# MatteoBattilana/CUDAVideoStream

Hardware: AMD Instinct MI355X
Metric: 1920×1080 RGB24 frames/sec (diff+threshold+pack); achieved HBM GB/s vs peak (higher is better)
Workload: dtype u8

## Files before the change

### cudavideostream_amd/csrc/core.hip

```cpp
#include <cmath>
#include <cstdio>
#include <cstdlib>
#include <cstring>
#include <new>
#include <string>
#include <vector>

#include "../../include/mi355diff.h"
#include "cwire_common.h"

using namespace mi355;

static inline size_t code_chunks(size_t max_batch) { return (max_batch + 2) / 3 + 1; }

namespace {

thread_local std::string g_err;

int fail(int code, const char *what, hipError_t e = hipSuccess) {
    char buf[512];
    if (e != hipSuccess)
        snprintf(buf, sizeof buf, "%s: %s (%s)", what, hipGetErrorName(e), hipGetErrorString(e));
    else
        snprintf(buf, sizeof buf, "%s", what);
    g_err = buf;
    return code;
}

#define HIP_TRY(expr)                                             \
    do {                                                          \
        hipError_t _e = (expr);                                   \
        if (_e != hipSuccess) return fail(MI355_ERR_HIP, #expr, _e); \
    } while (0)

}

struct mi355_core {
    mi355_config cfg{};
    int device = 0;
    uint32_t n = 0;
    uint32_t ntiles = 0;
    hipStream_t own_stream = nullptr;
    hipStream_t stream = nullptr;

    uint8_t *state = nullptr, *in = nullptr, *aux = nullptr, *vis = nullptr;
    uint4 *rec = nullptr, *meta = nullptr;
    uint32_t *codes = nullptr;
    uint32_t *groff = nullptr, *totals = nullptr;
    uint64_t scan_epoch = 0;
    uint32_t *offsets = nullptr;
    int32_t *one_xs = nullptr;
    uint8_t *one_diff = nullptr;
    int32_t *hist = nullptr, *thr = nullptr;
    uint32_t *red_bounds = nullptr;
    uint32_t *cw_cnt = nullptr;
    uint8_t *cw_rec = nullptr;
    uint64_t *cw_rec_pos = nullptr;
    uint64_t cw_rec_bytes = 0;
    static constexpr int kRecWords = 4;
    uint32_t *h_rec = nullptr;
    bool cw_warm = false;
    uint4 *cw_items = nullptr;
    uint32_t *cw_esc = nullptr;
    CwaFrame *cwa_ftab = nullptr;
    uint4 *cwa_chunk = nullptr;
    uint4 *cwa_dir = nullptr;
    uint32_t *cwb_hist = nullptr;
    uint8_t *gray1 = nullptr;
    size_t gray1_stride = 0;
    float *k9 = nullptr;
    float *kxk = nullptr;
    uint8_t *lut = nullptr;
    uint8_t *glyphs = nullptr;
    int nglyphs = 0, glyph_h = 0, glyph_w = 0;
    std::string charset;
    bool have_k9 = false, k9_sym = false;
    size_t workspace = 0;

    uint32_t *h_count = nullptr;

    static constexpr int kMaxSlots = 8;
    struct Slot {
        uint8_t *d_in = nullptr, *d_vis = nullptr;
        uint32_t *h_count = nullptr;
        hipEvent_t uploaded = nullptr, painted = nullptr, packed = nullptr, shown = nullptr;
        bool has_vis = false;
        bool compact = false;
        int64_t ticket = -1;
    };
    Slot slots[kMaxSlots];
    int nslots = 0;
    int64_t next_ticket = 0;
    hipStream_t up_stream = nullptr, down_stream = nullptr;

    struct LogSet {
        uint4 *rec = nullptr, *meta = nullptr;
        uint32_t *codes = nullptr, *groff = nullptr, *totals = nullptr;
        hipEvent_t packed = nullptr, expanded = nullptr;
        bool in_use = false;
    };
    static constexpr int kSets = 2;
    LogSet set[kSets];
    int flip = 0;
    hipStream_t side = nullptr;
    hipEvent_t side_done = nullptr;
    bool pipeline_ok = true;
    int median_rows = 0;
    uint32_t cu_count = 0;
    hipStream_t main2 = nullptr;
    hipEvent_t packed2[kSets] = {};
    static constexpr uint32_t kDensePct = 40;
    uint64_t *h_tot = nullptr;
    bool dense = false;
    bool filter_since_batch = false;
    hipEvent_t fork[kSets] = {};
    int parts_pending = -1;
    const void *fb_states = nullptr;
    size_t fb_stride = 0;

    static constexpr int kEvRing = 32, kEvPer = 6;
    bool timing = false;
    hipEvent_t ev[kEvRing][kEvPer] = {};
    bool ev_split[kEvRing] = {};
    int ev_head = 0, ev_count = 0;
    double ms_pack = 0, ms_scan = 0, ms_expand = 0, ms_total = 0;
    int launches = 0;
};

namespace mi355 {
int set_error(int code, const char *what) { return fail(code, what); }
hipStream_t core_stream(::mi355_core *c) {
    if (c->side_done && hipSetDevice(c->device) == hipSuccess && hipStreamWaitEvent(c->stream, c->side_done, 0) == hipSuccess)
        c->side_done = nullptr;
    return c->stream;
}
int core_device(const ::mi355_core *c) { return c->device; }
}

namespace {

hipError_t make_stream(const mi355_core *c, hipStream_t *s) {
    if (c->cfg.flags & MI355_FLAG_OWN_QUEUES) {
        int least = 0, greatest = 0;
        if (hipDeviceGetStreamPriorityRange(&least, &greatest) == hipSuccess && least != greatest)
            return hipStreamCreateWithPriority(s, hipStreamNonBlocking, least);
        (void)hipGetLastError();
    }
    return hipStreamCreateWithFlags(s, hipStreamNonBlocking);
}

template <class T>
int dev_alloc(mi355_core *c, T **p, size_t count) {
    const size_t bytes = count * sizeof(T);
    HIP_TRY(hipMalloc((void **)p, bytes ? bytes : 16));
    c->workspace += bytes;
    return MI355_OK;
}

int use_device(mi355_core *c, bool join = true, bool parts = true) {
    HIP_TRY(hipSetDevice(c->device));
    if (join && c->side_done) {
        HIP_TRY(hipStreamWaitEvent(c->stream, c->side_done, 0));
        c->side_done = nullptr;
        c->parts_pending = -1;
    }
    if (parts && c->parts_pending >= 0) {
        HIP_TRY(hipStreamWaitEvent(c->stream, c->packed2[c->parts_pending], 0));
        c->parts_pending = -1;
    }
    return MI355_OK;
}

int use_device_filter(mi355_core *c) {
    c->filter_since_batch = true;
    return use_device(c, false);
}

int harvest_timing(mi355_core *c, int keep = 0) {
    while (c->ev_count > keep) {
        hipEvent_t *e = c->ev[c->ev_head];
        HIP_TRY(hipEventSynchronize(e[4]));
        float a = 0, b = 0, d = 0, t = 0;
        HIP_TRY(hipEventElapsedTime(&a, e[0], e[1]));
        if (c->ev_split[c->ev_head]) {
            float a2 = 0;
            HIP_TRY(hipEventElapsedTime(&a2, e[0], e[5]));
            a = a2 > a ? a2 : a;
        }
        HIP_TRY(hipEventElapsedTime(&b, e[2], e[3]));
        HIP_TRY(hipEventElapsedTime(&d, e[3], e[4]));
        HIP_TRY(hipEventElapsedTime(&t, e[0], e[4]));
        c->ms_pack += a;
        c->ms_scan += b;
        c->ms_expand += d;
        c->ms_total += t;
        c->launches += 1;
        c->ev_head = (c->ev_head + 1) % mi355_core::kEvRing;
        c->ev_count -= 1;
    }
    return MI355_OK;
}

void build_heat_lut(uint8_t *lut) {
    for (int diff = 0; diff <= 765; diff++) {
        float diff1 = diff / (255.0 * 2.0);
        double r = sin(M_PI * diff1 - M_PI / 2.0) * 255.0;
        double g = sin(M_PI * diff1) * 255.0;
        double b = sin(M_PI * diff1 + M_PI / 2.0) * 255.0;
        r = r > 0.0 ? r : 0.0; r = r < 255.0 ? r : 255.0;
        g = g > 0.0 ? g : 0.0; g = g < 255.0 ? g : 255.0;
        b = b > 0.0 ? b : 0.0; b = b < 255.0 ? b : 255.0;
        lut[diff * 3 + 0] = (uint8_t)(int)b;
        lut[diff * 3 + 1] = (uint8_t)(int)g;
        lut[diff * 3 + 2] = (uint8_t)(int)r;
    }
}

int need_gray1(mi355_core *c) {
    if (c->gray1 || c->n == 0) return MI355_OK;
    c->gray1_stride = ((size_t)c->n / 3 + 15) & ~(size_t)15;
    return dev_alloc(c, &c->gray1, c->gray1_stride * (size_t)c->cfg.max_batch);
}

int clear_totals(mi355_core *c) {
    const size_t bytes = 2 * (size_t)c->cfg.max_batch * sizeof(uint32_t);
    HIP_TRY(hipMemsetAsync(c->totals, 0, bytes, c->stream));
    if (c->set[1].totals) HIP_TRY(hipMemsetAsync(c->set[1].totals, 0, bytes, c->stream));
    HIP_TRY(hipStreamSynchronize(c->stream));
    return MI355_OK;
}

int need_red_bounds(mi355_core *c) {
    if (c->red_bounds || c->n == 0) return MI355_OK;
    return dev_alloc(c, &c->red_bounds, (size_t)c->cfg.max_batch * red_bounds_per_frame(c->n));
}

int setup_pipeline(mi355_core *c) {
    if (c->side || !c->pipeline_ok) return MI355_OK;
    const size_t T = (size_t)c->cfg.max_batch, W = c->ntiles;
    mi355_core::LogSet &s0 = c->set[0], &s1 = c->set[1];
    s0.rec = c->rec; s0.codes = c->codes; s0.meta = c->meta; s0.groff = c->groff; s0.totals = c->totals;
    bool ok = true;
    ok = ok && hipMalloc((void **)&s1.rec, T * W * 1024) == hipSuccess;
    ok = ok && hipMalloc((void **)&s1.codes, code_chunks(T) * W * 1024) == hipSuccess;
    ok = ok && hipMalloc((void **)&s1.meta, T * W * 16) == hipSuccess;
    ok = ok && hipMalloc((void **)&s1.groff, T * expand_groups(c->ntiles) * 16) == hipSuccess;
    ok = ok && hipMalloc((void **)&s1.totals, (2 * T + 2) * sizeof(uint32_t)) == hipSuccess;
    ok = ok && hipMemsetAsync(s1.totals, 0, (2 * T + 2) * sizeof(uint32_t), c->stream) == hipSuccess &&
         hipStreamSynchronize(c->stream) == hipSuccess;
    ok = ok && make_stream(c, &c->side) == hipSuccess;
    ok = ok && make_stream(c, &c->main2) == hipSuccess;
    for (int i = 0; i < mi355_core::kSets && ok; i++) {
        const unsigned flags = hipEventDisableTiming | hipEventReleaseToDevice;
        ok = hipEventCreateWithFlags(&c->set[i].packed, flags) == hipSuccess &&
             hipEventCreateWithFlags(&c->set[i].expanded, flags) == hipSuccess &&
             hipEventCreateWithFlags(&c->packed2[i], flags) == hipSuccess &&
             hipEventCreateWithFlags(&c->fork[i], flags) == hipSuccess;
    }
    if (!ok) {
        (void)hipGetLastError();
        void *ptrs[] = {s1.rec, s1.codes, s1.meta, s1.groff, s1.totals};
        for (void *p : ptrs) if (p) (void)hipFree(p);
        s1.rec = nullptr; s1.meta = nullptr; s1.codes = s1.groff = s1.totals = nullptr;
        if (c->side) { (void)hipStreamDestroy(c->side); c->side = nullptr; }
        if (c->main2) { (void)hipStreamDestroy(c->main2); c->main2 = nullptr; }
        for (int i = 0; i < mi355_core::kSets; i++) {
            hipEvent_t *evs[] = {&c->set[i].packed, &c->set[i].expanded, &c->packed2[i], &c->fork[i]};
            for (hipEvent_t *e : evs) if (*e) { (void)hipEventDestroy(*e); *e = nullptr; }
        }
        c->pipeline_ok = false;
        return MI355_OK;
    }
    c->workspace += T * W * 1024 + code_chunks(T) * W * 1024 + T * W * 16 + T * expand_groups(c->ntiles) * 16 + (2 * T + 2) * 4;
    return MI355_OK;
}

struct CwireOut {
    uint64_t *frame_pos;
    uint8_t *cwire;
    uint64_t capacity;
};

CwireDirectArgs cwire_args(mi355_core *c, const CwireOut *cw, const uint32_t *d_offsets, uint32_t ntiles) {
    CwireDirectArgs x{};
    x.x.offsets = d_offsets;
    x.x.ntiles = ntiles;
    x.items = c->cw_items;
    x.esc = c->cw_esc;
    x.frame_pos = cw->frame_pos;
    x.cwire = cw->cwire;
    x.capacity = cw->capacity;
    return x;
}

int run_batch(mi355_core *c, bool pair, const void *d_cur, const void *d_prev, size_t stride,
              int nframes, void *d_offsets, void *d_xs, void *d_diff, size_t capacity,
              void *d_wire = nullptr, bool pipelined = false, const CwireOut *cw = nullptr, bool feedback = false,
              int seg = 0) {
    if (!c) return fail(MI355_ERR_INVALID, "null core");
    if (nframes < 0 || nframes > c->cfg.max_batch)
        return fail(MI355_ERR_INVALID, "nframes outside [0, max_batch]");
    if (!d_offsets) return fail(MI355_ERR_INVALID, "null d_offsets");
    if (nframes > 0 && c->n > 0 && (!d_cur || (pair && !d_prev)))
        return fail(MI355_ERR_INVALID, "null frame pointer");
    if (nframes > 0 && stride < c->n) return fail(MI355_ERR_INVALID, "stride_bytes < frame bytes");
    if (capacity > 0 && !d_wire && !cw && (!d_xs || !d_diff)) return fail(MI355_ERR_INVALID, "null output pointer");
    pipelined = pipelined && c->stream == c->own_stream && c->pipeline_ok && nframes > 0 && c->n > 0;
    const bool own = pipelined;
    if (c->filter_since_batch) pipelined = false;
    c->filter_since_batch = false;
    if (pipelined) {
        const bool same_states = feedback && c->fb_states == d_prev && c->fb_stride == stride;
        if (int rc = use_device(c, false, !same_states && (feedback || c->fb_states))) return rc;
        if (int rc = setup_pipeline(c)) return rc;
        pipelined = c->pipeline_ok;
    }
    if (pipelined && c->h_tot) {
        const uint64_t note = __atomic_load_n(c->h_tot, __ATOMIC_RELAXED);
        if (note >> 32) c->dense = (note & 0xffffffffull) * 100u > (uint64_t)mi355_core::kDensePct * (note >> 32) * c->n;
        if (c->dense) pipelined = false;
    }
    if (!pipelined)
        if (int rc = use_device(c)) return rc;
    c->fb_states = nullptr;
    if (nframes == 0 || c->n == 0) {
        HIP_TRY(hipMemsetAsync(d_offsets, 0, sizeof(uint32_t) * ((size_t)nframes + 1), c->stream));
        if (d_wire) {
            const size_t head = 4 * (size_t)nframes < capacity ? 4 * (size_t)nframes : capacity & ~(size_t)3;
            if (head) HIP_TRY(hipMemsetAsync(d_wire, 0, head, c->stream));
        }
        if (cw) HIP_TRY(launch_expand_cwire(cwire_args(c, cw, (const uint32_t *)d_offsets, 0u), nframes, c->stream));
        return MI355_OK;
    }
    hipEvent_t *tev = nullptr;
    if (c->timing) {
        if (int rc = harvest_timing(c, mi355_core::kEvRing - 1)) return rc;
        tev = c->ev[(c->ev_head + c->ev_count) % mi355_core::kEvRing];
    }
    mi355_core::LogSet one;
    one.rec = c->rec; one.codes = c->codes; one.meta = c->meta; one.groff = c->groff; one.totals = c->totals;
    mi355_core::LogSet &ls = pipelined ? c->set[c->flip] : one;
    hipStream_t tail = pipelined ? c->side : c->stream;
    if (pipelined && ls.in_use) HIP_TRY(hipStreamWaitEvent(c->stream, ls.expanded, 0));
    if (tev) HIP_TRY(hipEventRecord(tev[0], c->stream));
    PackArgs a{};
    a.cur = (const uint8_t *)d_cur;
    a.prev = seg ? nullptr : (const uint8_t *)d_prev;
    a.state = c->state;
    a.seg = seg;
    if (seg) a.states = (uint8_t *)const_cast<void *>(d_prev);
    a.stride = stride;
    a.n = c->n;
    a.nframes = nframes;
    a.thr = c->cfg.threshold;
    a.ntiles = c->ntiles;
    a.tile_begin = 0;
    a.tile_end = c->ntiles;
    a.rec = ls.rec;
    a.codes = ls.codes;
    a.codes_bytes = (uint32_t)(code_chunks((size_t)c->cfg.max_batch) * c->ntiles * 1024u);
    a.meta = ls.meta;
    a.rec_bytes = (uint32_t)((size_t)c->cfg.max_batch * c->ntiles * 1024u);
    a.meta_bytes = (uint32_t)((size_t)c->cfg.max_batch * c->ntiles * 16u);
    const bool aligned = (((uintptr_t)d_cur | (uintptr_t)d_prev | stride) & 15u) == 0 && 3 * (uint64_t)stride + c->n < (1ull << 32);
    bool pair_once = false;
    if (pair) {
        const int64_t d = (int64_t)((intptr_t)d_prev - (intptr_t)d_cur), st = (int64_t)stride, T = nframes;
        bool shared = false;
        const int64_t k0 = d / st;
        for (int64_t k = k0 - 1; k <= k0 + 1; k++)
            if (k > -T && k < T && (d - k * st < 0 ? k * st - d : d - k * st) < (int64_t)c->n) shared = true;
        pair_once = !shared;
    }
    const uint32_t k1_blocks = 4u * c->cu_count;
    const bool split = pipelined && c->main2 && c->ntiles >= 64;
    if (split) {
        const uint32_t cut = (c->ntiles / 2) & ~3u;
        uint32_t blocks0 = 0, blocks1 = 0;
        if (k1_blocks) {
            blocks0 = (uint32_t)((uint64_t)k1_blocks * cut / c->ntiles);
            if (blocks0 == 0) blocks0 = 1;
            blocks1 = k1_blocks > blocks0 ? k1_blocks - blocks0 : 1u;
        }
        HIP_TRY(hipEventRecord(c->fork[c->flip], c->stream));
        PackArgs a0 = a, a1 = a;
        a0.tile_end = cut;
        a1.tile_begin = cut;
        HIP_TRY(launch_diff_pack(a0, pair, aligned, pair_once, blocks0, c->stream, feedback));
        HIP_TRY(hipStreamWaitEvent(c->main2, c->fork[c->flip], 0));
        if (ls.in_use) HIP_TRY(hipStreamWaitEvent(c->main2, ls.expanded, 0));
        HIP_TRY(launch_diff_pack(a1, pair, aligned, pair_once, blocks1, c->main2, feedback));
        HIP_TRY(hipEventRecord(c->packed2[c->flip], c->main2));
        HIP_TRY(hipStreamWaitEvent(tail, c->packed2[c->flip], 0));
        if (tev) HIP_TRY(hipEventRecord(tev[5], c->main2));
        c->parts_pending = c->flip;
        if (feedback) { c->fb_states = d_prev; c->fb_stride = stride; }
    } else {
        HIP_TRY(launch_diff_pack(a, pair, aligned, pair_once, pipelined ? k1_blocks : 0u, c->stream, feedback));
    }
    if (tev) {
        HIP_TRY(hipEventRecord(tev[1], c->stream));
        c->ev_split[(c->ev_head + c->ev_count) % mi355_core::kEvRing] = split;
    }
    if (pipelined) {
        HIP_TRY(hipEventRecord(ls.packed, c->stream));
        HIP_TRY(hipStreamWaitEvent(tail, ls.packed, 0));
    }
    if (tev) HIP_TRY(hipEventRecord(tev[2], tail));
    if (next_scan_epoch(c->scan_epoch)) {
        HIP_TRY(hipStreamSynchronize(c->stream));
        if (c->side) HIP_TRY(hipStreamSynchronize(c->side));
        if (c->main2) HIP_TRY(hipStreamSynchronize(c->main2));
        if (int rc = clear_totals(c)) return rc;
    }
    uint64_t *const note = own && c->h_tot && c->pipeline_ok ? c->h_tot : nullptr;
    HIP_TRY(launch_scan(ls.meta, ls.groff, (uint64_t *)ls.totals, c->ntiles, nframes, (uint32_t *)d_offsets,
                        ls.totals + 2 * (size_t)c->cfg.max_batch, c->scan_epoch, note, tail));
    if (tev) HIP_TRY(hipEventRecord(tev[3], tail));
    ExpandArgs g{};
    g.rec = ls.rec;
    g.codes = ls.codes;
    g.meta = ls.meta;
    g.roff = ls.groff;
    g.offsets = (const uint32_t *)d_offsets;
    g.ntiles = c->ntiles;
    g.codes_bytes = a.codes_bytes;
    g.rec_bytes = a.rec_bytes;
    g.out_xs = (int32_t *)d_xs;
    g.out_diff = (uint8_t *)d_diff;
    g.wire = (uint8_t *)d_wire;
    g.capacity = capacity;
    if (cw) {
        CwireDirectArgs x = cwire_args(c, cw, g.offsets, c->ntiles);
        x.x = g;
        HIP_TRY(launch_expand_cwire(x, nframes, tail));
    } else {
        HIP_TRY(launch_expand(g, nframes, tail));
    }
    if (tev) {
        HIP_TRY(hipEventRecord(tev[4], tail));
        c->ev_count += 1;
    }
    if (pipelined) {
        HIP_TRY(hipEventRecord(ls.expanded, tail));
        ls.in_use = true;
        c->side_done = ls.expanded;
        c->flip ^= 1;
    }
    return MI355_OK;
}

}

extern "C" {

const char *mi355_last_error(void) { return g_err.c_str(); }

int mi355_abi_version(void) { return MI355_ABI_VERSION; }

int mi355_create(const mi355_config *cfg, mi355_core **out) {
    if (!cfg || !out) return fail(MI355_ERR_INVALID, "null argument");
    *out = nullptr;
    if (cfg->width < 0 || cfg->height < 0) return fail(MI355_ERR_INVALID, "negative frame size");
    if (cfg->threshold < 0 || cfg->threshold > 255) return fail(MI355_ERR_INVALID, "threshold outside 0..255");
    if (cfg->max_batch < 1) return fail(MI355_ERR_INVALID, "max_batch < 1");
    if (cfg->visualizer < 0 || cfg->visualizer > 5) return fail(MI355_ERR_INVALID, "unknown visualizer");
    if (cfg->flags & ~MI355_FLAG_OWN_QUEUES) return fail(MI355_ERR_INVALID, "flags: unknown bit (MI355_FLAG_OWN_QUEUES is the only flag of this version of the library)");
    const uint64_t n64 = 3ull * (uint64_t)cfg->width * (uint64_t)cfg->height;
    if (n64 >= (1ull << 31)) return fail(MI355_ERR_INVALID, "frame larger than 2 GiB");
    {
        const uint64_t tiles = (n64 + kTileBytes - 1) / kTileBytes, mb = (uint64_t)cfg->max_batch;
        const uint64_t chunks = mb > code_chunks((size_t)mb) ? mb : (uint64_t)code_chunks((size_t)mb);
        if (tiles * kTileBytes * chunks >= (1ull << 32))
            return fail(MI355_ERR_INVALID, "max_batch * frame bytes must stay below 2^32");
    }

    int ndev = 0;
    hipError_t e = hipGetDeviceCount(&ndev);
    if (e != hipSuccess || ndev <= 0)
        return fail(MI355_ERR_HIP, "no HIP device available (libmi355diff has no CPU fallback)", e);
    mi355_core *c = new (std::nothrow) mi355_core;
    if (!c) return fail(MI355_ERR_INVALID, "out of host memory");
    c->cfg = *cfg;
    if (const char *v = getenv("MI355_PIPELINE")) c->pipeline_ok = v[0] != '0';
    if (cfg->device >= 0) c->device = cfg->device;
    else if ((e = hipGetDevice(&c->device)) != hipSuccess) { delete c; return fail(MI355_ERR_HIP, "hipGetDevice", e); }
    if (c->device >= ndev) { delete c; return fail(MI355_ERR_INVALID, "device ordinal out of range"); }

    c->n = (uint32_t)n64;
    c->ntiles = (c->n + kTileBytes - 1) / kTileBytes;
    {
        hipDeviceProp_t prop{};
        if (hipGetDeviceProperties(&prop, c->device) == hipSuccess && prop.multiProcessorCount > 0) c->cu_count = (uint32_t)prop.multiProcessorCount;
    }
    const size_t T = (size_t)cfg->max_batch, W = c->ntiles, N = c->n;

    int rc = use_device(c);
    if (!rc) { e = make_stream(c, &c->own_stream); if (e != hipSuccess) rc = fail(MI355_ERR_HIP, "hipStreamCreate", e); }
    c->stream = c->own_stream;
    for (int i = 0; i < mi355_core::kEvRing * mi355_core::kEvPer && !rc; i++) { e = hipEventCreateWithFlags(&c->ev[i / mi355_core::kEvPer][i % mi355_core::kEvPer], hipEventDisableSystemFence); if (e != hipSuccess) rc = fail(MI355_ERR_HIP, "hipEventCreate", e); }
    if (!rc && (e = init_gray_table()) != hipSuccess) rc = fail(MI355_ERR_HIP, "init_gray_table", e);
    if (!rc) rc = dev_alloc(c, &c->state, N + 16);
    if (!rc) rc = dev_alloc(c, &c->in, N + 16);
    if (!rc) rc = dev_alloc(c, &c->aux, N + 16);
    if (!rc) rc = dev_alloc(c, &c->vis, N + 16);
    if (!rc) rc = dev_alloc(c, &c->rec, T * W * 64);
    if (!rc) rc = dev_alloc(c, &c->codes, code_chunks(T) * W * 256);
    if (!rc) rc = dev_alloc(c, &c->meta, T * W);
    if (!rc) rc = dev_alloc(c, &c->groff, T * expand_groups(c->ntiles) * 4);
    if (!rc) rc = dev_alloc(c, &c->totals, 2 * T + 2);
    if (!rc) { e = hipMemsetAsync(c->totals, 0, (2 * T + 2) * sizeof(uint32_t), c->own_stream); if (e != hipSuccess) rc = fail(MI355_ERR_HIP, "hipMemset", e); }
    if (!rc) rc = dev_alloc(c, &c->offsets, T + 1);
    if (!rc) rc = dev_alloc(c, &c->cw_cnt, (size_t)kCwireSlots);
    if (!rc) rc = dev_alloc(c, &c->cw_items, T * cwire_items_per_frame(c->ntiles));
    if (!rc) rc = dev_alloc(c, &c->cw_esc, T);
    if (!rc) rc = dev_alloc(c, &c->cwa_ftab, T);
    if (!rc) rc = dev_alloc(c, &c->cwa_chunk, T * cwa_chunks(c->n));
    if (!rc) rc = dev_alloc(c, &c->cwa_dir, T * cwa_tiles(c->n));
    if (!rc) rc = dev_alloc(c, &c->cwb_hist, T * kCwbWords);
    if (!rc) rc = dev_alloc(c, &c->one_xs, N + 4);
    if (!rc) rc = dev_alloc(c, &c->one_diff, N + 16);
    if (!rc) rc = dev_alloc(c, &c->hist, 256 * T);
    if (!rc) rc = dev_alloc(c, &c->thr, T);
    if (!rc) rc = dev_alloc(c, &c->k9, 9);
    if (!rc) rc = dev_alloc(c, &c->lut, 768 * 3);
    if (!rc) { e = hipHostMalloc((void **)&c->h_count, 2 * sizeof(uint32_t), hipHostMallocDefault); if (e != hipSuccess) rc = fail(MI355_ERR_HIP, "hipHostMalloc", e); }
    if (!rc) { e = hipHostMalloc((void **)&c->h_tot, sizeof(uint64_t), hipHostMallocDefault); if (e != hipSuccess) rc = fail(MI355_ERR_HIP, "hipHostMalloc", e); else *c->h_tot = 0; }
    if (!rc) { e = hipMemsetAsync(c->state, 0, N + 16, c->own_stream); if (e != hipSuccess) rc = fail(MI355_ERR_HIP, "hipMemset", e); }
    if (!rc) { e = hipStreamSynchronize(c->own_stream); if (e != hipSuccess) rc = fail(MI355_ERR_HIP, "hipStreamSynchronize", e); }
    if (!rc) {
        uint8_t lut[768 * 3] = {0};
        build_heat_lut(lut);
        e = hipMemcpy(c->lut, lut, sizeof lut, hipMemcpyHostToDevice);
        if (e != hipSuccess) rc = fail(MI355_ERR_HIP, "hipMemcpy(lut)", e);
    }
    if (!rc && cfg->visualizer == MI355_VIS_BINARIZE) rc = need_gray1(c);
    if (rc) { mi355_destroy(c); return rc; }
    *out = c;
    return MI355_OK;
}

void mi355_destroy(mi355_core *c) {
    if (!c) return;
    (void)hipSetDevice(c->device);
    if (c->nslots) (void)mi355_pipe_close(c);
    if (c->side) (void)hipStreamSynchronize(c->side);
    if (c->own_stream) (void)hipStreamSynchronize(c->own_stream);
    {
        mi355_core::LogSet &s1 = c->set[1];
        void *more[] = {s1.rec, s1.codes, s1.meta, s1.groff, s1.totals};
        for (void *p : more) if (p) (void)hipFree(p);
        for (auto &ls : c->set) {
            if (ls.packed) (void)hipEventDestroy(ls.packed);
            if (ls.expanded) (void)hipEventDestroy(ls.expanded);
        }
        if (c->side) (void)hipStreamDestroy(c->side);
        if (c->main2) { (void)hipStreamSynchronize(c->main2); (void)hipStreamDestroy(c->main2); }
        for (auto &e : c->packed2) if (e) (void)hipEventDestroy(e);
        for (auto &e : c->fork) if (e) (void)hipEventDestroy(e);
        if (c->h_tot) (void)hipHostFree(c->h_tot);
    }
    void *ptrs[] = {c->state, c->in, c->aux, c->vis, c->rec, c->codes, c->meta, c->groff, c->totals, c->offsets, c->one_xs, c->one_diff, c->hist, c->thr, c->k9,
                    c->lut, c->glyphs, c->kxk, c->gray1, c->red_bounds, c->cw_cnt, c->cw_items, c->cw_esc,
                    c->cwa_ftab, c->cwa_chunk, c->cwa_dir, c->cwb_hist, c->cw_rec, c->cw_rec_pos};
    for (void *p : ptrs) if (p) (void)hipFree(p);
    if (c->h_count) (void)hipHostFree(c->h_count);
    if (c->h_rec) (void)hipHostFree(c->h_rec);
    for (auto &slot : c->ev) for (auto &ev : slot) if (ev) (void)hipEventDestroy(ev);
    if (c->own_stream) (void)hipStreamDestroy(c->own_stream);
    delete c;
}

static int warm_exec(mi355_core *c);
static int need_exec_cwire(mi355_core *c);

int mi355_prepare(mi355_core *c, unsigned what) {
    if (!c) return fail(MI355_ERR_INVALID, "null core");
    if (what & ~(MI355_PREPARE_ALL | MI355_PREPARE_EXEC_CWIRE)) return fail(MI355_ERR_INVALID, "mi355_prepare: unknown bit in `what`");
    if (int rc = use_device(c)) return rc;
    if ((what & MI355_PREPARE_BATCHES) && c->n > 0) {
        if (int rc = setup_pipeline(c)) return rc;
    }
    if (what & MI355_PREPARE_GRAY_CHAIN)
        if (int rc = need_gray1(c)) return rc;
    if (what & MI355_PREPARE_RED_CLEAR)
        if (int rc = need_red_bounds(c)) return rc;
    if ((what & MI355_PREPARE_CONV_KXK) && !c->kxk)
        if (int rc = dev_alloc(c, &c->kxk, 81)) return rc;
    if ((what & MI355_PREPARE_EXEC) && c->n > 0 && c->nslots == 0)
        if (int rc = warm_exec(c)) return rc;
    if (what & MI355_PREPARE_EXEC_CWIRE)
        if (int rc = need_exec_cwire(c)) return rc;
    HIP_TRY(hipDeviceSynchronize());
    return MI355_OK;
}

size_t mi355_frame_bytes(const mi355_core *c) { return c ? c->n : 0; }
size_t mi355_workspace_bytes(const mi355_core *c) { return c ? c->workspace : 0; }

int mi355_set_stream(mi355_core *c, void *hip_stream) {
    if (!c) return fail(MI355_ERR_INVALID, "null core");
    if (int rc = use_device(c)) return rc;
    if (int rc = harvest_timing(c)) return rc;
    HIP_TRY(hipStreamSynchronize(c->stream));
    c->stream = (hipStream_t)hip_stream;
    return MI355_OK;
}

int mi355_use_own_stream(mi355_core *c) {
    if (!c) return fail(MI355_ERR_INVALID, "null core");
    if (int rc = use_device(c)) return rc;
    if (int rc = harvest_timing(c)) return rc;
    HIP_TRY(hipStreamSynchronize(c->stream));
    c->stream = c->own_stream;
    return MI355_OK;
}

int mi355_synchronize(mi355_core *c) {
    if (!c) return fail(MI355_ERR_INVALID, "null core");
    if (int rc = use_device(c)) return rc;
    HIP_TRY(hipStreamSynchronize(c->stream));
    return MI355_OK;
}

int mi355_set_option(mi355_core *c, int option, int value) {
    if (!c) return fail(MI355_ERR_INVALID, "null core");
    if (int rc = use_device(c)) return rc;
    HIP_TRY(hipStreamSynchronize(c->stream));
    switch (option) {
        case MI355_OPT_PIPELINE:
            if (value != 0 && value != 1) return fail(MI355_ERR_INVALID, "MI355_OPT_PIPELINE: 0 or 1");
            c->pipeline_ok = value == 1;
            return MI355_OK;
        case MI355_OPT_MEDIAN_ROWS:
            if (value < 0 || value > 60 || value % 5) return fail(MI355_ERR_INVALID, "MI355_OPT_MEDIAN_ROWS: 0 (default) or 5, 10, .. 60");
            c->median_rows = value;
            return MI355_OK;
        case MI355_OPT_SCAN_EPOCH_LEFT:
            if (value < 1 || value > (1 << 30)) return fail(MI355_ERR_INVALID, "MI355_OPT_SCAN_EPOCH_LEFT: 1..2^30");
            if (c->side) HIP_TRY(hipStreamSynchronize(c->side));
            if (c->main2) HIP_TRY(hipStreamSynchronize(c->main2));
            if (int rc = clear_totals(c)) return rc;
            c->scan_epoch = kEpochWrap - 1 - (uint64_t)value;
            return MI355_OK;
        default: return fail(MI355_ERR_INVALID, "unknown option");
    }
}

int mi355_get_option(mi355_core *c, int option, int *value) {
    if (!c || !value) return fail(MI355_ERR_INVALID, "null argument");
    switch (option) {
        case MI355_OPT_PIPELINE: *value = c->pipeline_ok ? 1 : 0; return MI355_OK;
        case MI355_OPT_MEDIAN_ROWS: *value = c->median_rows; return MI355_OK;
        case MI355_OPT_SCAN_EPOCH_LEFT: {
            const uint64_t left = kEpochWrap - 1 - c->scan_epoch;
            *value = left > (1ull << 30) ? (1 << 30) : (int)left;
            return MI355_OK;
        }
        default: return fail(MI355_ERR_INVALID, "unknown option");
    }
// ... 1818 lines not shown
```

### cudavideostream_amd/csrc/diff_pack.hip

```cpp
#include <cstdio>
#include <vector>

#include "cwire_common.h"
#include "pack_common.h"

namespace mi355 {

constexpr int kStreamPrefetch = 4;
template <bool PAIR>
struct PrefetchOf { static constexpr int value = PAIR ? 2 : kStreamPrefetch; };
static_assert(kStreamPrefetch % 2 == 0, "frames are processed in pairs");

typedef uint32_t u32x4 __attribute__((ext_vector_type(4)));
constexpr uint32_t kRsrcWord3 = 0x00020000u;
constexpr uint32_t kOOB = 0xFFFFFFFFu;

__device__ __forceinline__ __amdgpu_buffer_rsrc_t make_rsrc(const void *p, uint32_t bytes) {
    return __builtin_amdgcn_make_buffer_rsrc(const_cast<void *>(p), 0, (int)bytes, (int)kRsrcWord3);
}

struct LogOut {
    __amdgpu_buffer_rsrc_t codes, recs, meta;
};

constexpr int kStateLoadAux = 0, kStateStoreAux = 2;

template <bool HIGH>
__device__ __forceinline__ void compare_step(const uint4 c, uint4 &s, ThrConst tc, uint32_t (&dm)[4], uint32_t &m16) {
    const uint32_t cw[4] = {c.x, c.y, c.z, c.w};
    uint32_t sw[4] = {s.x, s.y, s.z, s.w};
    uint32_t fh[4];
#pragma unroll
    for (int k = 0; k < 4; k++) {
        uint32_t x;
        fh[k] = dword_flags<HIGH>(cw[k], sw[k], tc, x);
        const uint32_t mask = __builtin_amdgcn_perm(0u, 0u, fh[k]);
        dm[k] = bytes_sub_from_x(cw[k], sw[k], x, tc.h) & mask;
        sw[k] = bitop3<(TA & TC) | (TB & ~TC)>(cw[k], sw[k], mask);
    }
    s = make_uint4(sw[0], sw[1], sw[2], sw[3]);
    const uint32_t lo = __builtin_amdgcn_udot4(fh[1], tc.w1, __builtin_amdgcn_udot4(fh[0], tc.w0, 0u, false), false);
    const uint32_t hi = __builtin_amdgcn_udot4(fh[3], tc.w1, __builtin_amdgcn_udot4(fh[2], tc.w0, 0u, false), false);
    m16 = (lo + (hi << 8)) >> 7;
}

struct LogPos {
    uint32_t ptrC, roomC, ptrM, roomM;
};

__device__ __forceinline__ uint32_t emit_step(const uint32_t (&dm)[4], uint32_t m16, const LogOut &lg, LogPos &lp,
                                              uint32_t jump, uint32_t lane24, uint32_t &pc, uint32_t &pm) {
    const bool cand = m16 != 0u;
    const bool multi = (m16 & (m16 - 1u)) != 0u;
    const uint64_t bc = __ballot(cand), bm = __ballot(multi);
    const uint32_t rankC = __builtin_amdgcn_mbcnt_hi((uint32_t)(bc >> 32), __builtin_amdgcn_mbcnt_lo((uint32_t)bc, 0u));
    const uint32_t rankM = __builtin_amdgcn_mbcnt_hi((uint32_t)(bm >> 32), __builtin_amdgcn_mbcnt_lo((uint32_t)bm, 0u));
    const uint32_t nc = (uint32_t)__builtin_popcountll(bc), nm = (uint32_t)__builtin_popcountll(bm);
    pc = lp.ptrC;
    pm = lp.ptrM;
    if (nc == 0u) return 0u;
    if (nm > lp.roomM) { lp.ptrM += lp.roomM * 16u + jump; lp.roomM = 64u; }
    pm = lp.ptrM;
    if (nm == 64u) {
        const u32x4 v = {dm[0], dm[1], dm[2], dm[3]};
        __builtin_amdgcn_raw_buffer_store_b128(v, lg.recs, pm + rankM * 16u, 0, 0);
        lp.ptrM += 64u * 16u;
        lp.roomM -= 64u;
        return 64u | (64u << 16);
    }
    if (nc > lp.roomC) { lp.ptrC += lp.roomC * 4u + jump; lp.roomC = 256u; }
    pc = lp.ptrC;
    const uint32_t one = __builtin_amdgcn_sad_u8((dm[0] | dm[1]) | (dm[2] | dm[3]), 0u, 0u);
    const uint32_t code = m16 | ((multi ? rankM : one) << 16) | lane24;
    __builtin_amdgcn_raw_buffer_store_b32(code, lg.codes, cand ? pc + rankC * 4u : kOOB, 0, 0);
    const u32x4 v = {dm[0], dm[1], dm[2], dm[3]};
    __builtin_amdgcn_raw_buffer_store_b128(v, lg.recs, multi ? pm + rankM * 16u : kOOB, 0, 0);
    lp.ptrC += nc * 4u;
    lp.roomC -= nc;
    lp.ptrM += nm * 16u;
    lp.roomM -= nm;
    return nc | (nm << 16);
}

template <bool PAIR, bool FAST>
struct Group {
    static constexpr int kPrefetch = PrefetchOf<PAIR>::value;
    uint4 c[kPrefetch];
    uint4 p[kPrefetch];

    template <bool ONCE, bool FB = false>
    __device__ __forceinline__ void load_desc(__amdgpu_buffer_rsrc_t cur, __amdgpu_buffer_rsrc_t prev, const uint32_t (&voff)[kPrefetch]) {
#pragma unroll
        for (int d = 0; d < kPrefetch; d++) {
            const u32x4 v = __builtin_amdgcn_raw_buffer_load_b128(cur, voff[d], 0, ONCE ? 2 : 0);
            c[d] = make_uint4(v.x, v.y, v.z, v.w);
            if (PAIR) {
                const u32x4 w = __builtin_amdgcn_raw_buffer_load_b128(prev, voff[d], 0, FB ? kStateLoadAux : (ONCE ? 2 : 0));
                p[d] = make_uint4(w.x, w.y, w.z, w.w);
            }
        }
    }

    __device__ __forceinline__ void load(const PackArgs &a, uint32_t byte_off, int t0, int valid, const uint8_t *cur0,
                                         const uint8_t *prev0, const uint8_t *cur_last, const uint8_t *prev_last) {
        const int last = a.nframes - 1;
#pragma unroll
        for (int d = 0; d < kPrefetch; d++) {
            const bool in = t0 + d <= last;
            const uint8_t *cb = uniform_ptr(in ? cur0 + (size_t)d * a.stride : cur_last);
            c[d] = load16<FAST, !PAIR>(cb + byte_off, valid);
            if (PAIR) {
                const uint8_t *pb = uniform_ptr(in ? prev0 + (size_t)d * a.stride : prev_last);
                p[d] = load16<FAST>(pb + byte_off, valid);
            }
        }
    }
};

struct StateOut {
    __amdgpu_buffer_rsrc_t desc;
    const uint32_t *voff;
    uint8_t *base;
};

template <bool FAST>
__device__ __forceinline__ void store_state(const PackArgs &a, const StateOut &so, int d, uint4 st, uint32_t m16, int valid) {
    if (FAST) {
        const u32x4 v = {st.x, st.y, st.z, st.w};
        __builtin_amdgcn_raw_buffer_store_b128(v, so.desc, m16 != 0u ? so.voff[d] : kOOB, 0, kStateStoreAux);
    } else {
        store16_bytes(so.base + (size_t)d * a.stride, st, m16 != 0u ? valid : 0);
    }
}

struct Seg {
    int32_t left;
    int32_t next;
    uint32_t chg;
    uint32_t byte_off;
};

template <bool FAST>
__device__ __forceinline__ uint4 load_seg_state(const PackArgs &a, int32_t k, uint32_t byte_off, int valid, bool want) {
    const uint8_t *base = uniform_ptr(a.states + (size_t)k * a.stride);
    if (FAST) {
        const u32x4 v = __builtin_amdgcn_raw_buffer_load_b128(make_rsrc(base, a.n), want ? byte_off : kOOB, 0, kStateLoadAux);
        return make_uint4(v.x, v.y, v.z, v.w);
    }
    return load16_bytes(base + byte_off, want ? valid : 0);
}

template <bool FAST>
__device__ __forceinline__ void store_seg_state(const PackArgs &a, int32_t k, const Seg &sg, uint4 st, int valid) {
    uint8_t *base = const_cast<uint8_t *>(uniform_ptr(a.states + (size_t)k * a.stride));
    if (FAST) {
        const u32x4 v = {st.x, st.y, st.z, st.w};
        __builtin_amdgcn_raw_buffer_store_b128(v, make_rsrc(base, a.n), sg.chg != 0u ? sg.byte_off : kOOB, 0, kStateStoreAux);
    } else {
        store16_bytes(base + sg.byte_off, st, sg.chg != 0u ? valid : 0);
    }
}

template <bool FAST>
__device__ __forceinline__ void exchange_state(const PackArgs &a, Seg &sg, uint4 &st, const uint4 &ns, bool first, int valid) {
    if (sg.next > 0) store_seg_state<FAST>(a, sg.next - 1, sg, st, valid);
    st = first ? ns : load_seg_state<FAST>(a, sg.next, sg.byte_off, valid, true);
    sg.next += 1;
    sg.left = a.seg;
    sg.chg = 0u;
}

template <bool PAIR, bool FAST, bool HIGH, bool FB = false, bool SEG = false>
__device__ __forceinline__ void pack_group(const PackArgs &a, const Group<PAIR, FAST> &g, int t0, uint4 &st,
                                           LogPos &lp, uint32_t tile, ThrConst tc, int lane, const LogOut &lg,
                                           const StateOut *so = nullptr, int valid = 16, Seg *sg = nullptr,
                                           const uint4 *ns = nullptr) {
    bool first = true;
    constexpr int kPrefetch = PrefetchOf<PAIR>::value;
    uint4 meta = make_uint4(0, 0, 0, 0);
    const uint32_t lane24 = ((uint32_t)lane << 24) | (tile << 30);
    const uint32_t jump = (a.ntiles - 1u) * 1024u;
#pragma unroll
    for (int d = 0; d < kPrefetch; d += 2) {
        const int t = t0 + d;
        if (t >= a.nframes) break;
        const bool two = t + 1 < a.nframes;
        uint32_t dm0[4], m0, m1 = 0, pc0, pm0, pc1 = 0, pm1 = 0;
        if (PAIR) st = g.p[d];
        if (SEG) {
            if (sg->left == 0) { exchange_state<FAST>(a, *sg, st, *ns, first, valid); first = false; }
            sg->left -= 1;
        }
        compare_step<HIGH>(g.c[d], st, tc, dm0, m0);
        if (SEG) sg->chg |= m0;
        if (FB) store_state<FAST>(a, *so, d, st, m0, valid);
        const uint32_t c0 = emit_step(dm0, m0, lg, lp, jump, lane24, pc0, pm0);
        uint32_t c1 = 0;
        if (two) {
            if (PAIR) st = g.p[d + 1];
            if (SEG) {
                if (sg->left == 0) { exchange_state<FAST>(a, *sg, st, *ns, first, valid); first = false; }
                sg->left -= 1;
            }
            uint32_t dm1[4];
            compare_step<HIGH>(g.c[d + 1], st, tc, dm1, m1);
            if (SEG) sg->chg |= m1;
            if (FB) store_state<FAST>(a, *so, d + 1, st, m1, valid);
            c1 = emit_step(dm1, m1, lg, lp, jump, lane24, pc1, pm1);
        }
        const uint32_t both = (uint32_t)__builtin_popcount(m0) | ((uint32_t)__builtin_popcount(m1) << 16);
        const uint32_t tot = (uint32_t)__builtin_amdgcn_readlane(wave_inclusive_scan((int)both), 63);
        write_lane(meta.x, pc0, d);
        write_lane(meta.y, pm0, d);
        write_lane(meta.z, tot & 0xffffu, d);
        write_lane(meta.w, c0, d);
        write_lane(meta.x, pc1, d + 1);
        write_lane(meta.y, pm1, d + 1);
        write_lane(meta.z, tot >> 16, d + 1);
        write_lane(meta.w, c1, d + 1);
    }
    const uint32_t moff = (__umul24((uint32_t)t0 + (uint32_t)lane, a.ntiles) + tile) * 16u;
    const u32x4 mv = {meta.x, meta.y, meta.z, meta.w};
    __builtin_amdgcn_raw_buffer_store_b128(mv, lg.meta, (lane < kPrefetch && t0 + lane < a.nframes) ? moff : kOOB, 0, 0);
}

template <bool PAIR, bool FAST, bool HIGH, bool ONCE, bool FB = false, bool SEG = false>
__device__ __forceinline__ void pack_tile(const PackArgs &a, uint32_t tile, uint32_t byte_off,
                                          int valid, int lane) {
    const int T = a.nframes;
    const ThrConst tc = make_thr((uint32_t)a.thr);
    const LogOut lg{make_rsrc(a.codes, a.codes_bytes), make_rsrc(a.rec, a.rec_bytes), make_rsrc(a.meta, a.meta_bytes)};

    uint4 st = make_uint4(0, 0, 0, 0);
    if (!PAIR && !SEG) st = load16<FAST>(a.state + byte_off, valid);

    Group<PAIR, FAST> ga, gb;
    LogPos lp{tile * 1024u, 256u, tile * 1024u, 64u};
    constexpr int kPrefetch = PrefetchOf<PAIR>::value;
    const size_t gstep = (size_t)kPrefetch * a.stride;
    Seg sg{0, 0, 0u, byte_off};
    int32_t pk = 0, pf = 0;
    uint4 na = st, nb = st;
    auto prefetch_state = [&](int t0) {
        const uint4 v = load_seg_state<FAST>(a, pk, byte_off, valid, pf < t0 + kPrefetch && pf < T);
        while (pf < t0 + kPrefetch) { pf += a.seg; pk += 1; }
        return v;
    };
    if (FAST) {
        uint32_t voff[kPrefetch];
#pragma unroll
        for (int d = 0; d < kPrefetch; d++) voff[d] = byte_off + (uint32_t)d * (uint32_t)a.stride;
        const uint8_t *cb = a.cur, *pb = a.prev;
        int64_t left = (int64_t)(T - 1) * (int64_t)a.stride + (int64_t)a.n;
        auto desc = [&](const uint8_t *base) {
            const uint32_t bytes = left <= 0 ? 0u : (left > 0xffffffffll ? 0xffffffffu : (uint32_t)left);
            return make_rsrc(base, bytes);
        };
        if (FB) {
            StateOut sa{desc(pb), voff, nullptr}, sb = sa;
            ga.template load_desc<ONCE, true>(desc(cb), sa.desc, voff);
            for (int t0 = 0;;) {
                cb += gstep; pb += gstep; left -= (int64_t)gstep;
                sb.desc = desc(pb);
                gb.template load_desc<ONCE, true>(desc(cb), sb.desc, voff);
                pack_group<PAIR, FAST, HIGH, true>(a, ga, t0, st, lp, tile, tc, lane, lg, &sa);
                t0 += kPrefetch;
                if (t0 >= T) break;
                cb += gstep; pb += gstep; left -= (int64_t)gstep;
                sa.desc = desc(pb);
                ga.template load_desc<ONCE, true>(desc(cb), sa.desc, voff);
                pack_group<PAIR, FAST, HIGH, true>(a, gb, t0, st, lp, tile, tc, lane, lg, &sb);
                t0 += kPrefetch;
                if (t0 >= T) break;
            }
            return;
        }
        if (SEG) {
            na = prefetch_state(0);
            ga.template load_desc<ONCE>(desc(cb), desc(cb), voff);
            for (int t0 = 0;;) {
                cb += gstep; left -= (int64_t)gstep;
                nb = prefetch_state(t0 + kPrefetch);
                gb.template load_desc<ONCE>(desc(cb), desc(cb), voff);
                pack_group<PAIR, FAST, HIGH, false, true>(a, ga, t0, st, lp, tile, tc, lane, lg, nullptr, valid, &sg, &na);
                t0 += kPrefetch;
                if (t0 >= T) break;
                cb += gstep; left -= (int64_t)gstep;
                na = prefetch_state(t0 + kPrefetch);
                ga.template load_desc<ONCE>(desc(cb), desc(cb), voff);
                pack_group<PAIR, FAST, HIGH, false, true>(a, gb, t0, st, lp, tile, tc, lane, lg, nullptr, valid, &sg, &nb);
                t0 += kPrefetch;
                if (t0 >= T) break;
            }
            store_seg_state<FAST>(a, sg.next - 1, sg, st, valid);
            return;
        }
        ga.template load_desc<ONCE>(desc(cb), desc(pb), voff);
        for (int t0 = 0;;) {
            cb += gstep; if (PAIR) pb += gstep; left -= (int64_t)gstep;
            gb.template load_desc<ONCE>(desc(cb), desc(pb), voff);
            pack_group<PAIR, FAST, HIGH>(a, ga, t0, st, lp, tile, tc, lane, lg);
            t0 += kPrefetch;
            if (t0 >= T) break;
            cb += gstep; if (PAIR) pb += gstep; left -= (int64_t)gstep;
            ga.template load_desc<ONCE>(desc(cb), desc(pb), voff);
            pack_group<PAIR, FAST, HIGH>(a, gb, t0, st, lp, tile, tc, lane, lg);
            t0 += kPrefetch;
            if (t0 >= T) break;
        }
        if (!PAIR) *reinterpret_cast<uint4 *>(a.state + byte_off) = st;
        return;
    }
    const uint8_t *cur_last = a.cur + (size_t)(T - 1) * a.stride, *prev_last = PAIR ? a.prev + (size_t)(T - 1) * a.stride : nullptr;
    const uint8_t *cp = a.cur, *pp = a.prev;
    if (FB) {
        StateOut sa{lg.meta, nullptr, const_cast<uint8_t *>(pp) + byte_off}, sb = sa;
        ga.load(a, byte_off, 0, valid, cp, pp, cur_last, prev_last);
        for (int t0 = 0;;) {
            cp += gstep; pp += gstep;
            sb.base = const_cast<uint8_t *>(pp) + byte_off;
            gb.load(a, byte_off, t0 + kPrefetch, valid, cp, pp, cur_last, prev_last);
            pack_group<PAIR, FAST, HIGH, true>(a, ga, t0, st, lp, tile, tc, lane, lg, &sa, valid);
            t0 += kPrefetch;
            if (t0 >= T) break;
            cp += gstep; pp += gstep;
            sa.base = const_cast<uint8_t *>(pp) + byte_off;
            ga.load(a, byte_off, t0 + kPrefetch, valid, cp, pp, cur_last, prev_last);
            pack_group<PAIR, FAST, HIGH, true>(a, gb, t0, st, lp, tile, tc, lane, lg, &sb, valid);
            t0 += kPrefetch;
            if (t0 >= T) break;
        }
        return;
    }
    if (SEG) {
        na = prefetch_state(0);
        ga.load(a, byte_off, 0, valid, cp, pp, cur_last, prev_last);
        for (int t0 = 0;;) {
            cp += gstep;
            nb = prefetch_state(t0 + kPrefetch);
            gb.load(a, byte_off, t0 + kPrefetch, valid, cp, pp, cur_last, prev_last);
            pack_group<PAIR, FAST, HIGH, false, true>(a, ga, t0, st, lp, tile, tc, lane, lg, nullptr, valid, &sg, &na);
            t0 += kPrefetch;
            if (t0 >= T) break;
            cp += gstep;
            na = prefetch_state(t0 + kPrefetch);
            ga.load(a, byte_off, t0 + kPrefetch, valid, cp, pp, cur_last, prev_last);
            pack_group<PAIR, FAST, HIGH, false, true>(a, gb, t0, st, lp, tile, tc, lane, lg, nullptr, valid, &sg, &nb);
            t0 += kPrefetch;
            if (t0 >= T) break;
        }
        store_seg_state<FAST>(a, sg.next - 1, sg, st, valid);
        return;
    }
    ga.load(a, byte_off, 0, valid, cp, pp, cur_last, prev_last);
    for (int t0 = 0;;) {
        cp += gstep; if (PAIR) pp += gstep;
        gb.load(a, byte_off, t0 + kPrefetch, valid, cp, pp, cur_last, prev_last);
        pack_group<PAIR, FAST, HIGH>(a, ga, t0, st, lp, tile, tc, lane, lg);
        t0 += kPrefetch;
        if (t0 >= T) break;
        cp += gstep; if (PAIR) pp += gstep;
        ga.load(a, byte_off, t0 + kPrefetch, valid, cp, pp, cur_last, prev_last);
        pack_group<PAIR, FAST, HIGH>(a, gb, t0, st, lp, tile, tc, lane, lg);
        t0 += kPrefetch;
        if (t0 >= T) break;
    }

    if (!PAIR) {
        if (FAST) *reinterpret_cast<uint4 *>(a.state + byte_off) = st;
        else store16_bytes(a.state + byte_off, st, valid);
    }
}

template <bool PAIR, bool ALIGNED, bool HIGH, bool ONCE = !PAIR, bool FB = false, bool SEG = false>
__global__ __launch_bounds__(256) void k_diff_pack(const PackArgs a) {
    static_assert(!FB || PAIR, "feedback write-back is a form of pair mode");
    static_assert(!SEG || !PAIR, "segments are a form of stream mode");
    const int lane = threadIdx.x & 63;
    const uint32_t wave = (uint32_t)__builtin_amdgcn_readfirstlane((int)(threadIdx.x >> 6));
    for (uint32_t tile = a.tile_begin + blockIdx.x * kWavesPerBlock + wave; tile < a.tile_end; tile += gridDim.x * kWavesPerBlock) {
        const uint32_t tile_off = tile * kTileBytes;
        const uint32_t byte_off = tile_off + (uint32_t)lane * 16u;
        if (ALIGNED && tile_off + kTileBytes <= a.n) {
            pack_tile<PAIR, true, HIGH, ONCE, FB, SEG>(a, tile, byte_off, 16, lane);
        } else {
            const int valid = byte_off < a.n ? (int)min(16u, a.n - byte_off) : 0;
            pack_tile<PAIR, false, HIGH, ONCE, FB, SEG>(a, tile, byte_off, valid, lane);
        }
    }
}
// ... 713 lines not shown
```

### cudavideostream_amd/csrc/internal.h

```cpp
#ifndef MI355_INTERNAL_H_
#define MI355_INTERNAL_H_

#include <hip/hip_runtime.h>
#include <stddef.h>
#include <stdint.h>

namespace mi355 {

constexpr uint32_t kTileBytes = 1024;
constexpr uint32_t kWavesPerBlock = 4;

struct PackArgs {
    const uint8_t *cur;
    const uint8_t *prev;
    union {
        uint8_t *state;
        uint8_t *states;
    };
    size_t stride;
    uint32_t n;
    int32_t nframes;
    int32_t thr;
    uint32_t ntiles;
    uint32_t tile_begin;
    uint32_t tile_end;
    uint32_t *codes;
    uint4 *rec;
    uint4 *meta;
    uint32_t codes_bytes;
    uint32_t rec_bytes;
    uint32_t meta_bytes;
    int32_t seg;
};
static_assert(sizeof(PackArgs) == 96, "see above");

struct ExpandArgs {
    const uint32_t *codes;
    const uint4 *rec;
    const uint4 *meta;
    const uint32_t *roff;
    const uint32_t *offsets;
    uint32_t ntiles;
    uint32_t codes_bytes;
    uint32_t rec_bytes;
    int32_t *out_xs;
    uint8_t *out_diff;
    uint8_t *wire;
    size_t capacity;
};

}
struct mi355_core;
namespace mi355 {
int set_error(int code, const char *what);
hipStream_t core_stream(::mi355_core *c);
int core_device(const ::mi355_core *c);

hipError_t launch_diff_pack(const PackArgs &a, bool pair, bool aligned, bool pair_once ,
                            uint32_t max_blocks , hipStream_t s,
                            bool feedback = false );
uint32_t expand_groups(uint32_t ntiles);
constexpr int kTotalBits = 31;
constexpr uint64_t kEpochWrap = 1ull << (64 - kTotalBits);
inline bool next_scan_epoch(uint64_t &epoch) {
    if (++epoch < kEpochWrap) return false;
    epoch = 1;
    return true;
}
hipError_t launch_scan(const uint4 *meta, uint32_t *roff, uint64_t *totals , uint32_t ntiles,
                       int nframes, uint32_t *offsets, uint32_t *ticket ,
                       uint64_t epoch ,
                       uint64_t *note , hipStream_t s);
hipError_t launch_expand(const ExpandArgs &a, int nframes, hipStream_t s);
__host__ __device__ uint32_t cwire_items_per_frame(uint32_t ntiles);
struct CwireDirectArgs {
    ExpandArgs x;
    uint4 *items;
    uint32_t *esc;
    uint64_t *frame_pos;
    uint8_t *cwire;
    uint64_t capacity;
};
hipError_t launch_expand_cwire(const CwireDirectArgs &a, int nframes, hipStream_t s);

constexpr int kMaxParts = 64;
struct MergeArgs {
    const uint32_t *part_off;
    const int32_t *xs_all;
    const uint8_t *diff_all;
    int32_t *out_xs;
    uint8_t *out_diff;
    size_t capacity;
    int32_t nparts, nframes;
    uint32_t part_base[kMaxParts];
    int32_t xs_bias[kMaxParts];
};
hipError_t launch_apply(uint8_t *frame, uint32_t nbytes, const void *xs, const void *diff,
                        const uint32_t *d_offsets, int t, uint32_t host_count, hipStream_t s);
hipError_t launch_apply_all(uint8_t *frame, uint32_t nbytes, const int32_t *xs, const uint8_t *diff,
                            const uint32_t *d_offsets, int nframes, hipStream_t s);
hipError_t launch_apply_multi(uint8_t *states, size_t stride, uint32_t nbytes, const uint32_t *d_offsets, const int32_t *xs,
                              const uint8_t *diff, int nstreams, hipStream_t s);
constexpr int kApplyMultiWireStreams = 128;
struct ApplyMultiWireArgs {
    int32_t first, count;
    uint64_t pos[kApplyMultiWireStreams];
    uint64_t cum[kApplyMultiWireStreams + 1];
};
hipError_t launch_apply_multi_wire(uint8_t *states, size_t stride, uint32_t nbytes, const uint8_t *wire,
                                   const ApplyMultiWireArgs &h, hipStream_t s);
hipError_t launch_apply_multi_strided(uint8_t *states, size_t stride, uint32_t nbytes, const uint32_t *d_offsets, const int32_t *xs,
                                      const uint8_t *diff, int nstreams, int nframes, int t, hipStream_t s);
hipError_t launch_apply_multi_show(const uint8_t *states, size_t stride, uint32_t nbytes, uint8_t *out, size_t out_stride,
                                   int nstreams, int nframes, int t, hipStream_t s);
hipError_t launch_export(const uint32_t *offsets, const int32_t *xs, const uint8_t *diff, int32_t *h_xs,
                         uint8_t *h_diff, uint32_t *h_count, hipStream_t s);
hipError_t launch_export_record(const uint64_t *frame_pos, const uint8_t *rec, uint64_t rec_bytes, uint32_t *h_record,
                                uint32_t *h_words, hipStream_t s);
hipError_t launch_merge(const MergeArgs &a, uint32_t *out_offsets, hipStream_t s);
constexpr int kCwireSlots = 8192;
int cwire_blocks_per_frame(int nframes);
hipError_t launch_cwire_encode(const uint32_t *offsets, const int32_t *xs, const uint8_t *diff, uint64_t entries_capacity,
                               int nframes, uint32_t *cnt , uint64_t *frame_pos, uint8_t *out,
                               uint64_t capacity_bytes, hipStream_t s);
constexpr int kCwireDecodeFrames = 64;
struct CwireFrame {
    uint64_t pos;
    uint32_t n, e;
    uint32_t out;
    uint32_t pad;
};
struct CwireDecodeArgs {
    const uint8_t *cwire;
    uint32_t *offsets;
    int32_t *xs;
    uint8_t *diff;
    uint64_t capacity;
    int32_t first_frame;
    CwireFrame frame[kCwireDecodeFrames];
};
hipError_t launch_cwire_decode(const CwireDecodeArgs &a, int nframes, hipStream_t s);
constexpr uint32_t kCwaChunk = 4096;
constexpr uint32_t kCwaTile = 4096;
constexpr int kCwaTableFrames = 128;
struct CwaFrame {
    uint64_t pos;
    uint32_t n, e;
    uint32_t cbase, nc;
};
struct CwaArgs {
    const uint8_t *cwire;
    CwaFrame *ftab;
    uint4 *chunk;
    uint4 *dir;
    uint8_t *state;
    uint8_t *out;
    size_t stride;
    uint32_t n;
    uint32_t ntiles;
};
struct CwaTableArgs {
    int32_t first;
    CwaFrame frame[kCwaTableFrames];
};
uint32_t cwa_chunks(uint32_t n);
uint32_t cwa_tiles(uint32_t nbytes);
hipError_t launch_cwire_apply(const CwaArgs &a, const CwaFrame *frames, int nframes, hipStream_t s);
hipError_t launch_cwire_apply_multi(const CwaArgs &a, const CwaFrame *records, int nstreams, hipStream_t s);
hipError_t launch_cwire_apply_multi_stream(const CwaArgs &a, const CwaFrame *records, int nstreams, int nframes, size_t out_stride,
                                           hipStream_t s);
struct CwcOut {
    uint32_t *offsets;
    uint64_t *frame_pos;
    uint8_t *cwire;
    int32_t *xs;
    uint8_t *diff;
    uint64_t capacity;
};
hipError_t launch_cwire_coalesce(const CwaArgs &a, const CwaFrame *records, int nstreams, int nframes, const CwcOut &o, bool cwire,
                                 hipStream_t s);
constexpr int kCwbInitStreams = 128;
constexpr uint32_t kCwbBudget = 256, kCwbThr = 257, kCwbWords = 258;
struct CwbInitArgs {
    int32_t first;
    uint32_t thr0;
    uint32_t budget[kCwbInitStreams];
};
// ... 73 lines not shown
```

Baseline: 564,300.

## Give each tile a contiguous worst-case log region and drop room checks

```diff
diff --git a/cudavideostream_amd/csrc/core.hip b/cudavideostream_amd/csrc/core.hip
--- a/cudavideostream_amd/csrc/core.hip
+++ b/cudavideostream_amd/csrc/core.hip
@@ -11,7 +11,14 @@
 
 using namespace mi355;
 
-static inline size_t code_chunks(size_t max_batch) { return (max_batch + 2) / 3 + 1; }
+struct LogGeometry {
+    uint32_t code_stride, rec_stride;
+    size_t codes_bytes, rec_bytes;
+};
+static inline LogGeometry log_geometry(size_t max_batch, size_t ntiles) {
+    const size_t cs = max_batch * 256, rs = max_batch * 1024;
+    return LogGeometry{(uint32_t)cs, (uint32_t)rs, cs * ntiles, rs * ntiles};
+}
 
 namespace {
 
@@ -239,10 +246,11 @@
     if (c->side || !c->pipeline_ok) return MI355_OK;
     const size_t T = (size_t)c->cfg.max_batch, W = c->ntiles;
     mi355_core::LogSet &s0 = c->set[0], &s1 = c->set[1];
+    const LogGeometry lg = log_geometry(T, W);
     s0.rec = c->rec; s0.codes = c->codes; s0.meta = c->meta; s0.groff = c->groff; s0.totals = c->totals;
     bool ok = true;
-    ok = ok && hipMalloc((void **)&s1.rec, T * W * 1024) == hipSuccess;
-    ok = ok && hipMalloc((void **)&s1.codes, code_chunks(T) * W * 1024) == hipSuccess;
+    ok = ok && hipMalloc((void **)&s1.rec, lg.rec_bytes) == hipSuccess;
+    ok = ok && hipMalloc((void **)&s1.codes, lg.codes_bytes) == hipSuccess;
     ok = ok && hipMalloc((void **)&s1.meta, T * W * 16) == hipSuccess;
     ok = ok && hipMalloc((void **)&s1.groff, T * expand_groups(c->ntiles) * 16) == hipSuccess;
     ok = ok && hipMalloc((void **)&s1.totals, (2 * T + 2) * sizeof(uint32_t)) == hipSuccess;
@@ -271,7 +279,7 @@
         c->pipeline_ok = false;
         return MI355_OK;
     }
-    c->workspace += T * W * 1024 + code_chunks(T) * W * 1024 + T * W * 16 + T * expand_groups(c->ntiles) * 16 + (2 * T + 2) * 4;
+    c->workspace += lg.rec_bytes + lg.codes_bytes + T * W * 16 + T * expand_groups(c->ntiles) * 16 + (2 * T + 2) * 4;
     return MI355_OK;
 }
 
@@ -358,9 +366,12 @@
     a.tile_end = c->ntiles;
     a.rec = ls.rec;
     a.codes = ls.codes;
-    a.codes_bytes = (uint32_t)(code_chunks((size_t)c->cfg.max_batch) * c->ntiles * 1024u);
+    const LogGeometry geo = log_geometry((size_t)c->cfg.max_batch, c->ntiles);
+    a.codes_bytes = (uint32_t)geo.codes_bytes;
     a.meta = ls.meta;
-    a.rec_bytes = (uint32_t)((size_t)c->cfg.max_batch * c->ntiles * 1024u);
+    a.rec_bytes = (uint32_t)geo.rec_bytes;
+    a.code_stride = geo.code_stride;
+    a.rec_stride = geo.rec_stride;
     a.meta_bytes = (uint32_t)((size_t)c->cfg.max_batch * c->ntiles * 16u);
     const bool aligned = (((uintptr_t)d_cur | (uintptr_t)d_prev | stride) & 15u) == 0 && 3 * (uint64_t)stride + c->n < (1ull << 32);
     bool pair_once = false;
@@ -470,8 +481,7 @@
     if (n64 >= (1ull << 31)) return fail(MI355_ERR_INVALID, "frame larger than 2 GiB");
     {
         const uint64_t tiles = (n64 + kTileBytes - 1) / kTileBytes, mb = (uint64_t)cfg->max_batch;
-        const uint64_t chunks = mb > code_chunks((size_t)mb) ? mb : (uint64_t)code_chunks((size_t)mb);
-        if (tiles * kTileBytes * chunks >= (1ull << 32))
+        if (tiles * kTileBytes * (mb > 2 ? mb : 2) >= (1ull << 32))
             return fail(MI355_ERR_INVALID, "max_batch * frame bytes must stay below 2^32");
     }
 
@@ -504,8 +514,9 @@
     if (!rc) rc = dev_alloc(c, &c->in, N + 16);
     if (!rc) rc = dev_alloc(c, &c->aux, N + 16);
     if (!rc) rc = dev_alloc(c, &c->vis, N + 16);
-    if (!rc) rc = dev_alloc(c, &c->rec, T * W * 64);
-    if (!rc) rc = dev_alloc(c, &c->codes, code_chunks(T) * W * 256);
+    const LogGeometry lg = log_geometry(T, W);
+    if (!rc) rc = dev_alloc(c, &c->rec, lg.rec_bytes / 16);
+    if (!rc) rc = dev_alloc(c, &c->codes, lg.codes_bytes / 4);
     if (!rc) rc = dev_alloc(c, &c->meta, T * W);
     if (!rc) rc = dev_alloc(c, &c->groff, T * expand_groups(c->ntiles) * 4);
     if (!rc) rc = dev_alloc(c, &c->totals, 2 * T + 2);
diff --git a/cudavideostream_amd/csrc/diff_pack.hip b/cudavideostream_amd/csrc/diff_pack.hip
--- a/cudavideostream_amd/csrc/diff_pack.hip
+++ b/cudavideostream_amd/csrc/diff_pack.hip
@@ -45,11 +45,11 @@
 }
 
 struct LogPos {
-    uint32_t ptrC, roomC, ptrM, roomM;
+    uint32_t ptrC, ptrM;
 };
 
 __device__ __forceinline__ uint32_t emit_step(const uint32_t (&dm)[4], uint32_t m16, const LogOut &lg, LogPos &lp,
-                                              uint32_t jump, uint32_t lane24, uint32_t &pc, uint32_t &pm) {
+                                              uint32_t lane24, uint32_t &pc, uint32_t &pm) {
     const bool cand = m16 != 0u;
     const bool multi = (m16 & (m16 - 1u)) != 0u;
     const uint64_t bc = __ballot(cand), bm = __ballot(multi);
@@ -59,26 +59,19 @@
     pc = lp.ptrC;
     pm = lp.ptrM;
     if (nc == 0u) return 0u;
-    if (nm > lp.roomM) { lp.ptrM += lp.roomM * 16u + jump; lp.roomM = 64u; }
-    pm = lp.ptrM;
     if (nm == 64u) {
         const u32x4 v = {dm[0], dm[1], dm[2], dm[3]};
         __builtin_amdgcn_raw_buffer_store_b128(v, lg.recs, pm + rankM * 16u, 0, 0);
         lp.ptrM += 64u * 16u;
-        lp.roomM -= 64u;
         return 64u | (64u << 16);
     }
-    if (nc > lp.roomC) { lp.ptrC += lp.roomC * 4u + jump; lp.roomC = 256u; }
-    pc = lp.ptrC;
     const uint32_t one = __builtin_amdgcn_sad_u8((dm[0] | dm[1]) | (dm[2] | dm[3]), 0u, 0u);
     const uint32_t code = m16 | ((multi ? rankM : one) << 16) | lane24;
     __builtin_amdgcn_raw_buffer_store_b32(code, lg.codes, cand ? pc + rankC * 4u : kOOB, 0, 0);
     const u32x4 v = {dm[0], dm[1], dm[2], dm[3]};
     __builtin_amdgcn_raw_buffer_store_b128(v, lg.recs, multi ? pm + rankM * 16u : kOOB, 0, 0);
     lp.ptrC += nc * 4u;
-    lp.roomC -= nc;
     lp.ptrM += nm * 16u;
-    lp.roomM -= nm;
     return nc | (nm << 16);
 }
 
@@ -178,8 +171,9 @@
     bool first = true;
     constexpr int kPrefetch = PrefetchOf<PAIR>::value;
     uint4 meta = make_uint4(0, 0, 0, 0);
+    lp.ptrC = (uint32_t)__builtin_amdgcn_readfirstlane((int)lp.ptrC);
+    lp.ptrM = (uint32_t)__builtin_amdgcn_readfirstlane((int)lp.ptrM);
     const uint32_t lane24 = ((uint32_t)lane << 24) | (tile << 30);
-    const uint32_t jump = (a.ntiles - 1u) * 1024u;
 #pragma unroll
     for (int d = 0; d < kPrefetch; d += 2) {
         const int t = t0 + d;
@@ -194,7 +188,7 @@
         compare_step<HIGH>(g.c[d], st, tc, dm0, m0);
         if (SEG) sg->chg |= m0;
         if (FB) store_state<FAST>(a, *so, d, st, m0, valid);
-        const uint32_t c0 = emit_step(dm0, m0, lg, lp, jump, lane24, pc0, pm0);
+        const uint32_t c0 = emit_step(dm0, m0, lg, lp, lane24, pc0, pm0);
         uint32_t c1 = 0;
         if (two) {
             if (PAIR) st = g.p[d + 1];
@@ -206,7 +200,7 @@
             compare_step<HIGH>(g.c[d + 1], st, tc, dm1, m1);
             if (SEG) sg->chg |= m1;
             if (FB) store_state<FAST>(a, *so, d + 1, st, m1, valid);
-            c1 = emit_step(dm1, m1, lg, lp, jump, lane24, pc1, pm1);
+            c1 = emit_step(dm1, m1, lg, lp, lane24, pc1, pm1);
         }
         const uint32_t both = (uint32_t)__builtin_popcount(m0) | ((uint32_t)__builtin_popcount(m1) << 16);
         const uint32_t tot = (uint32_t)__builtin_amdgcn_readlane(wave_inclusive_scan((int)both), 63);
@@ -235,7 +229,7 @@
     if (!PAIR && !SEG) st = load16<FAST>(a.state + byte_off, valid);
 
     Group<PAIR, FAST> ga, gb;
-    LogPos lp{tile * 1024u, 256u, tile * 1024u, 64u};
+    LogPos lp{tile * a.code_stride, tile * a.rec_stride};
     constexpr int kPrefetch = PrefetchOf<PAIR>::value;
     const size_t gstep = (size_t)kPrefetch * a.stride;
     Seg sg{0, 0, 0u, byte_off};
diff --git a/cudavideostream_amd/csrc/internal.h b/cudavideostream_amd/csrc/internal.h
--- a/cudavideostream_amd/csrc/internal.h
+++ b/cudavideostream_amd/csrc/internal.h
@@ -31,8 +31,10 @@
     uint32_t rec_bytes;
     uint32_t meta_bytes;
     int32_t seg;
-};
-static_assert(sizeof(PackArgs) == 96, "see above");
+    uint32_t code_stride;
+    uint32_t rec_stride;
+};
+static_assert(sizeof(PackArgs) == 104, "kernel arguments: no padding but the union's");
 
 struct ExpandArgs {
     const uint32_t *codes;
```

Result: faster. 591,400 (median of 6 runs) (+4.8%).
